# insight-platform/Similari

Hardware: NVIDIA H100
Metric: pair_associations_per_sec (higher is better)
Workload: dtype f32

## Files before the change

similari_b200/csrc/kernels_feat_tc.cu:

```cuda
#include <cuda.h>
#include <cuda_bf16.h>
#include <cuda_runtime.h>
#include <stdint.h>

#include <algorithm>
#include <cstdlib>
#include <cstring>

#include "sb_engine.cuh"
#include "sb_tc.cuh"

namespace sb {

constexpr int TC_STAGES = 4;
constexpr int TC_STAGE_BYTES = TC_A_BYTES + TC_B_BYTES;

struct TcHdr { int scene, m0, ncols_left, m, det_base, col0, epoch, vis_lbase, vis_lcap, pad; };
struct TcSmem {
  unsigned char stage[TC_STAGES][TC_STAGE_BYTES];
  VisColMeta meta[4][TC_BN];
  VisRowMeta rowm[4][TC_BM];
  float colb[4][TC_BN];
  unsigned int colvalid[4][TC_BN / 32];
  TcHdr hdr[4];
// ... 149 lines not shown
        const int total = __shfl_sync(0xffffffffu, incl, 31);
        int base = 0;
        if (lane == 31) base = atomicAdd(&f.vis_cnt[h.scene], total);
        base = __shfl_sync(0xffffffffu, base, 31);
        int pos = base + incl - cnt;
#pragma unroll
        for (int hr = 0; hr < 2; ++hr) {
#pragma unroll
          for (int w = 0; w < 4; ++w) {
            unsigned int kk = keep[w] & (hr ? 0xccccccccu : 0x33333333u);
            while (kk) {
              const int b = __ffs(kk) - 1;
              kk &= kk - 1;
              if (pos < h.vis_lcap) {
                const int i = w * 32 + b;
                const VisColMeta cm = gmeta[8 * (i >> 2) + q2 + (i & 1)];
                VisPair vp;
                vp.g = g[hr]; vp.row = cm.row; vp.scene = h.scene; vp.outcol = cm.outcol;
                f.vis_pairs[h.vis_lbase + pos] = vp;
              }
              ++pos;
            }
          }
        }
      }
      __syncwarp();
      if (lane == 0) mbar_arrive(&S.meta_empty[ms]);
    }
  }
  __syncthreads();
  cluster_sync_all();
}

constexpr int SA_BN = 128;
constexpr int SA_KMAX = 8;
constexpr int SA_A_BLOCK = TC_BM * TC_BK * 2;
constexpr int SA_B_STAGE = SA_BN * TC_BK * 2;
constexpr int SA_STAGES = 5;
constexpr int SA_SLABS = 4;
struct SaHdr { int scene, m0, ncols, m, det_base, col0, epoch, vis_lbase, vis_lcap, unit, last, pad; };
struct SaSmem {
  unsigned char a[SA_KMAX][SA_A_BLOCK];
  unsigned char b[SA_STAGES][SA_B_STAGE];
  VisColMeta meta[SA_SLABS][SA_BN];
  float colb[SA_SLABS][SA_BN];
  unsigned int colvalid[SA_SLABS][SA_BN / 32];
  SaHdr hdr[SA_SLABS];
  unsigned long long a_full[SA_KMAX];
  unsigned long long a_empty;
  unsigned long long full_bar[SA_STAGES];
  unsigned long long empty_bar[SA_STAGES];
  unsigned long long meta_full[SA_SLABS];
  unsigned long long meta_empty[SA_SLABS];
};
static_assert(sizeof(SaSmem) + 1024 <= 227 * 1024, "A-stationary screen kernel exceeds the shared memory of an SM");
constexpr int kScreenStationaryMaxD8 = SA_KMAX * TC_BK;

template <bool COSINE>
__global__ void __launch_bounds__(TC_THREADS, 1)
vis_screen_sa_kernel(const __grid_constant__ CUtensorMap mapA, const __grid_constant__ CUtensorMap mapB, Params p,
                     TrackStore ts, Frame f, const TcTile* units, int n_units_host, const int* n_units_dev, int ucols,
                     const VisColMeta* colmeta, const VisColGeo* colgeo, const VisRowMeta* rowmeta, const float* colb,
                     const unsigned int* colvalid) {
  const int n_units = n_units_dev ? *n_units_dev : n_units_host;
  extern __shared__ unsigned char smem_raw_[];
  SaSmem& S = *reinterpret_cast<SaSmem*>(smem_raw_ + ((1024u - (smem_u32(smem_raw_) & 1023u)) & 1023u));
  const int warp = threadIdx.x >> 5, lane = threadIdx.x & 31;
  const int K = p.max_obs;
  const int KB = (p.d8 + TC_BK - 1) / TC_BK;
  const uint32_t crank = cluster_rank();
  if (threadIdx.x == 0) {
    for (int kb = 0; kb < SA_KMAX; ++kb) mbar_init(&S.a_full[kb], 1);
    mbar_init(&S.a_empty, 2);
    for (int s = 0; s < SA_STAGES; ++s) { mbar_init(&S.full_bar[s], 1); mbar_init(&S.empty_bar[s], 2); }
    for (int b = 0; b < SA_SLABS; ++b) { mbar_init(&S.meta_full[b], 1); mbar_init(&S.meta_empty[b], 4); }
    asm volatile("fence.mbarrier_init.release.cluster;" ::: "memory");
  }
  __syncthreads();
  cluster_sync_all();

  if (warp < 4) {
    asm volatile("setmaxnreg.dec.sync.aligned.u32 40;");
    if (warp == 0 && lane == 0) {
      asm volatile("prefetch.tensormap [%0];" ::"l"((uint64_t)&mapA) : "memory");
      asm volatile("prefetch.tensormap [%0];" ::"l"((uint64_t)&mapB) : "memory");
      int seq = 0, gk = 0, unit = 0;
      for (int u = (int)(blockIdx.x >> 1); u < n_units; u += (int)(gridDim.x >> 1), ++unit) {
        const TcTile tl = units[u];
        const SceneDesc sc = f.scenes[tl.scene];
        const int m0 = tl.m0 + (int)crank * TC_BM;
        const int rowA = sc.det_base + m0;
        const int cols = min(ucols, sc.nb * K - tl.c0);
        const int nct = (cols + SA_BN - 1) / SA_BN;
        const int rowB = sc.slot * ts.track_cap * K + tl.c0;
        if (unit > 0) mbar_wait(&S.a_empty, (unit - 1) & 1);
        if (nct == 1) mbar_arrive(&S.a_empty);
        for (int ct = 0; ct < nct; ++ct, ++seq) {
          const int g = seq % SA_SLABS;
          mbar_wait(&S.meta_empty[g], ((seq / SA_SLABS) & 1) ^ 1);
          SaHdr h;
          h.scene = tl.scene; h.m0 = m0; h.ncols = min(SA_BN, cols - ct * SA_BN); h.m = sc.m; h.det_base = sc.det_base;
          h.col0 = sc.col_off + tl.c0 + ct * SA_BN; h.epoch = (int)sc.epoch; h.vis_lbase = sc.vis_lbase;
          h.vis_lcap = sc.vis_lcap; h.unit = unit; h.last = ct + 2 >= nct; h.pad = 0;
          S.hdr[g] = h;
          mbar_expect_tx(&S.meta_full[g], (uint32_t)(sizeof(VisColMeta) * SA_BN + 4 * SA_BN + SA_BN / 8));
          bulk_load(S.meta[g], colmeta + h.col0, (uint32_t)(sizeof(VisColMeta) * SA_BN), &S.meta_full[g]);
          bulk_load(S.colb[g], colb + h.col0, 4 * SA_BN, &S.meta_full[g]);
          bulk_load(S.colvalid[g], colvalid + (h.col0 >> 5), SA_BN / 8, &S.meta_full[g]);
          for (int kb = 0; kb < KB; ++kb, ++gk) {
            if (ct == 0) {
              mbar_expect_tx(&S.a_full[kb], SA_A_BLOCK);
              tma_load_2d(S.a[kb], &mapA, kb * TC_BK, rowA, &S.a_full[kb]);
            }
            const int s = gk % SA_STAGES;
            mbar_wait(&S.empty_bar[s], ((gk / SA_STAGES) & 1) ^ 1);
            mbar_expect_tx(&S.full_bar[s], SA_B_STAGE);
            tma_load_2d_mc(S.b[s] + crank * (SA_B_STAGE / 2), &mapB, kb * TC_BK, rowB + ct * SA_BN + (int)crank * (SA_BN / 2),
                           &S.full_bar[s], (uint16_t)0x3);
          }
        }
      }
      for (int e = 0; e < 2; ++e, ++seq) {
        const int g = seq % SA_SLABS;
        mbar_wait(&S.meta_empty[g], ((seq / SA_SLABS) & 1) ^ 1);
        S.hdr[g].scene = -1 - e;
        mbar_arrive(&S.meta_full[g]);
      }
    }
  } else {
    asm volatile("setmaxnreg.inc.sync.aligned.u32 232;");
    const int wg = (warp >> 2) - 1;
    const int rr[2] = {(warp & 3) * 16 + (lane >> 2), (warp & 3) * 16 + (lane >> 2) + 8};
    const int q2 = 2 * (lane & 3);
    const bool geo = p.n_constraints > 0;
    const bool elected = (threadIdx.x & 127) == 0;
    for (int pos = wg;; pos += 2) {
      const int ms = pos % SA_SLABS;
      mbar_wait(&S.meta_full[ms], (pos / SA_SLABS) & 1);
      const SaHdr h = S.hdr[ms];
      if (pos > 0) wg2_bar_sync(1 + (pos & 1));
      if (h.scene < 0) {
        if (h.scene == -1) wg2_bar_arrive(1 + ((pos + 1) & 1));
        break;
      }
      float rowk[2][2];
      bool row_ok[2][2];
#pragma unroll
      for (int hh = 0; hh < 2; ++hh)
#pragma unroll
        for (int hr = 0; hr < 2; ++hr) {
          const int m = h.m0 + 64 * hh + rr[hr];
          const VisRowMeta rm = rowmeta[h.det_base + m];
          rowk[hh][hr] = rm.rowk;
          row_ok[hh][hr] = m < h.m && rm.ok;
        }

      float acc[128];
      {
        const int g0 = pos * KB;
        int stage = g0 % SA_STAGES;
        uint32_t phase = (g0 / SA_STAGES) & 1;
        int prev = -1;
        auto release = [&](int s) {
          if (elected)
            for (uint32_t r = 0; r < 2; ++r) mbar_arrive_cluster(cluster_addr(&S.empty_bar[s], r));
        };
        for (int kb = 0; kb < KB; ++kb) {
          mbar_wait(&S.a_full[kb], (uint32_t)h.unit & 1u);
          mbar_wait(&S.full_bar[stage], phase);
          const uint32_t a0 = smem_u32(S.a[kb]);
          const uint32_t b0 = smem_u32(S.b[stage]);
          wgmma_fence();
#pragma unroll
          for (int k = 0; k < TC_BK / 16; ++k) {
            const uint32_t acc_on = (kb | k) != 0 ? 1u : 0u;
// ... 43 lines not shown
        keep[2 * hh + 1] &= colm[1] & rowm;
      }
      if (geo) {
        float cx[2][2], cy[2][2], cr[2][2];
#pragma unroll
        for (int hh = 0; hh < 2; ++hh)
#pragma unroll
          for (int hr = 0; hr < 2; ++hr) {
            cx[hh][hr] = 0.0f; cy[hh][hr] = 0.0f; cr[hh][hr] = 0.0f;
            if (row_ok[hh][hr]) {
              const size_t g = (size_t)h.det_base + h.m0 + 64 * hh + rr[hr];
              cx[hh][hr] = f.c_box[g * 6]; cy[hh][hr] = f.c_box[g * 6 + 1]; cr[hh][hr] = f.c_radius[g];
            }
          }
#pragma unroll
        for (int w = 0; w < 4; ++w) {
          unsigned int kk = keep[w];
          while (kk) {
            const int b = __ffs(kk) - 1;
            kk &= kk - 1;
            const int i = (w & 1) * 32 + b, hh = w >> 1;
            const bool r8 = (i >> 1) & 1;
            const int col = 8 * (i >> 2) + q2 + (i & 1);
            const VisColGeo cg = colgeo[h.col0 + col];
            if (!compat_ok(p, (unsigned int)h.epoch, cg.tep, r8 ? cx[hh][1] : cx[hh][0], r8 ? cy[hh][1] : cy[hh][0],
                           r8 ? cr[hh][1] : cr[hh][0], cg.tx, cg.ty, cg.tr))
              keep[w] &= ~(1u << b);
          }
        }
      }
      int cnt = 0;
#pragma unroll
      for (int w = 0; w < 4; ++w) cnt += __popc(keep[w]);
      if (__any_sync(0xffffffffu, cnt != 0)) {
        int incl = cnt;
#pragma unroll
        for (int o = 1; o < 32; o <<= 1) {
          int tt = __shfl_up_sync(0xffffffffu, incl, o);
          if (lane >= o) incl += tt;
        }
        const int total = __shfl_sync(0xffffffffu, incl, 31);
        int base = 0;
        if (lane == 31) base = atomicAdd(&f.vis_cnt[h.scene], total);
        base = __shfl_sync(0xffffffffu, base, 31);
        int at = base + incl - cnt;
#pragma unroll
        for (int hh = 0; hh < 2; ++hh) {
#pragma unroll
          for (int hr = 0; hr < 2; ++hr) {
            const int g = h.det_base + h.m0 + 64 * hh + rr[hr];
#pragma unroll
            for (int w = 0; w < 2; ++w) {
              unsigned int kk = keep[2 * hh + w] & (hr ? 0xccccccccu : 0x33333333u);
              while (kk) {
                const int b = __ffs(kk) - 1;
                kk &= kk - 1;
                if (at < h.vis_lcap) {
                  const int i = w * 32 + b;
                  const VisColMeta cm = gmeta[8 * (i >> 2) + q2 + (i & 1)];
                  VisPair vp;
                  vp.g = g; vp.row = cm.row; vp.scene = h.scene; vp.outcol = cm.outcol;
                  f.vis_pairs[h.vis_lbase + at] = vp;
                }
                ++at;
              }
            }
          }
        }
      }
      __syncwarp();
      if (lane == 0) mbar_arrive(&S.meta_empty[ms]);
    }
  }
  __syncthreads();
  cluster_sync_all();
}

__device__ __forceinline__ float reduce_add8_tc(const float* t) {
  float q0 = t[0] + t[4], q1 = t[1] + t[5], q2 = t[2] + t[6], q3 = t[3] + t[7];
  float d0 = q0 + q2, d1 = q1 + q3;
  return d0 + d1;
}

constexpr int RF_WARPS = 4;
constexpr int RF_SEG = 64;
constexpr int RF_PITCH = RF_SEG + 1;

template <bool TAIL>
__device__ __forceinline__ void refine_load_a(const float* __restrict__ a, int blk, int D, float* av) {
  if (!TAIL) {
    const float4 a0 = *reinterpret_cast<const float4*>(a + blk * 8);
    const float4 a1 = *reinterpret_cast<const float4*>(a + blk * 8 + 4);
    av[0] = a0.x; av[1] = a0.y; av[2] = a0.z; av[3] = a0.w; av[4] = a1.x; av[5] = a1.y; av[6] = a1.z; av[7] = a1.w;
  } else {
#pragma unroll
    for (int l = 0; l < 8; ++l) av[l] = blk * 8 + l < D ? a[blk * 8 + l] : 0.0f;
  }
}
template <bool COSINE>
__device__ __forceinline__ float refine_block_sum(const float* av, const float* __restrict__ b, int blk) {
  const float4 b0 = *reinterpret_cast<const float4*>(b + blk * 8);
  const float4 b1 = *reinterpret_cast<const float4*>(b + blk * 8 + 4);
  const float bb[8] = {b0.x, b0.y, b0.z, b0.w, b1.x, b1.y, b1.z, b1.w};
  float t[8];
#pragma unroll
  for (int l = 0; l < 8; ++l) {
    if (COSINE) t[l] = av[l] * bb[l];
    else { const float df = av[l] - bb[l]; t[l] = df * df; }
  }
  return reduce_add8_tc(t);
}

template <bool COSINE, bool TAIL, int RP>
__global__ void __launch_bounds__(RF_WARPS * 32, RP == 32 ? 6 : 8) vis_refine_kernel(Params p, TrackStore ts, Frame f, int* nan_flag) {
  __shared__ float s_bs[RF_WARPS][RP][RF_PITCH];
  const int scene = blockIdx.y;
  if (f.vis_mode[scene] != 0) return;
  const SceneDesc sc = f.scenes[scene];
  const int lane = threadIdx.x & 31, w = threadIdx.x >> 5;
  const int n_pairs = min(f.vis_cnt[scene], sc.vis_lcap);
  const int nblk = p.d8 / 8;
  const int D = p.feature_dim;
  float (*bs)[RF_PITCH] = s_bs[w];
  float vmax = nanf("");
  for (;;) {
    int i0 = 0;
    if (lane == 0) i0 = atomicAdd(f.refine_next + scene, RP);
    i0 = __shfl_sync(0xffffffffu, i0, 0);
    if (i0 >= n_pairs) break;
    const int npair = min(RP, n_pairs - i0);
    VisPair mine;
    mine.g = 0; mine.row = 0; mine.scene = 0; mine.outcol = 0;
    if (lane < npair) mine = f.vis_pairs[sc.vis_lbase + i0 + lane];
    float acc = 0.0f;
    for (int seg0 = 0; seg0 < nblk; seg0 += RF_SEG) {
      const int segn = min(RF_SEG, nblk - seg0);
      int g_prev = -1;
      float av[RF_SEG / 32][8];
#pragma unroll 4
      for (int pp = 0; pp < npair; ++pp) {
        const int g = __shfl_sync(0xffffffffu, mine.g, pp);
        const int row = __shfl_sync(0xffffffffu, mine.row, pp);
        const float* b = ts.feat + (size_t)row * p.d8;
        if (g != g_prev) {
          const float* a = f.in_feat + (size_t)g * D;
#pragma unroll
          for (int h = 0; h < RF_SEG / 32; ++h)
            if (h * 32 + lane < segn) refine_load_a<TAIL>(a, seg0 + h * 32 + lane, D, av[h]);
          g_prev = g;
        }
#pragma unroll
        for (int h = 0; h < RF_SEG / 32; ++h) {
          const int j = h * 32 + lane;
          if (j < segn) bs[pp][j] = refine_block_sum<COSINE>(av[h], b, seg0 + j);
        }
      }
      __syncwarp();
      if (lane < npair)
        for (int j = 0; j < segn; ++j) acc = acc + bs[lane][j];
      __syncwarp();
    }
    if (lane < npair) {
      float v = nanf("");
      if (COSINE) {
        const float d = acc / sqrtf(f.c_norm2[mine.g] * ts.fnorm2[mine.row]);
        if (d >= p.visual_threshold) v = 1.0f - d;
      } else {
        const float d = sqrtf(acc);
        if (d <= p.visual_threshold) v = d;
      }
      f.vis_val[sc.vis_lbase + i0 + lane] = v;
      if (!is_nan(v) && !(v <= vmax)) vmax = v;
      if (nan_flag && is_nan(v)) nan_flag[scene] = 1;
    }
  }
  unsigned int u = 0u;
  if (!is_nan(vmax)) {
    u = __float_as_uint(vmax);
    u = (u & 0x80000000u) ? ~u : (u | 0x80000000u);
  }
#pragma unroll
  for (int o = 16; o > 0; o >>= 1) u = max(u, __shfl_xor_sync(0xffffffffu, u, o));
  if (lane == 0 && u != 0u) atomicMax(f.scene_max + scene, u);
}

constexpr int RA_WARPS = 6;
constexpr int RA_STAGES = 3;
constexpr int RA_PAIRS = 2;
constexpr int RA_SEGF = RF_SEG * 8;
constexpr int RA_STAGE_FLOATS = RA_PAIRS * 2 * RA_SEGF;

__device__ __forceinline__ void cp_async16(void* smem_dst, const void* gsrc) {
  asm volatile("cp.async.cg.shared.global [%0], [%1], 16;" ::"r"(smem_u32(smem_dst)), "l"(gsrc) : "memory");
}
__device__ __forceinline__ void cp_async_commit() { asm volatile("cp.async.commit_group;" ::: "memory"); }
template <int N>
__device__ __forceinline__ void cp_async_wait() { asm volatile("cp.async.wait_group %0;" ::"n"(N) : "memory"); }

template <bool COSINE>
__global__ void __launch_bounds__(RA_WARPS * 32) vis_refine_async_kernel(Params p, TrackStore ts, Frame f, int* nan_flag) {
  extern __shared__ __align__(16) unsigned char ra_smem[];
  const int scene = blockIdx.y;
  if (f.vis_mode[scene] != 0) return;
  const SceneDesc sc = f.scenes[scene];
  const int lane = threadIdx.x & 31, w = threadIdx.x >> 5;
  float* stage0 = reinterpret_cast<float*>(ra_smem) + (size_t)w * (RA_STAGES * RA_STAGE_FLOATS + 32 * RF_PITCH);
  float (*bs)[RF_PITCH] = reinterpret_cast<float (*)[RF_PITCH]>(stage0 + RA_STAGES * RA_STAGE_FLOATS);
  const int n_pairs = min(f.vis_cnt[scene], sc.vis_lcap);
  const int nblk = p.d8 / 8;
  const int D = p.feature_dim;
  float vmax = nanf("");
  for (;;) {
    int i0 = 0;
    if (lane == 0) i0 = atomicAdd(f.refine_next + scene, 32);
    i0 = __shfl_sync(0xffffffffu, i0, 0);
    if (i0 >= n_pairs) break;
// ... 45 lines not shown
          const int pp = st * RA_PAIRS + pi;
          if (pp < npair) {
            const float* sa = src + (pi * 2) * RA_SEGF;
            const float* sb2 = sa + RA_SEGF;
#pragma unroll
            for (int h = 0; h < RF_SEG / 32; ++h) {
              const int j = h * 32 + lane;
              if (j < segn) {
                const float4 a0 = *reinterpret_cast<const float4*>(sa + j * 4);
                const float4 a1 = *reinterpret_cast<const float4*>(sa + (RF_SEG + j) * 4);
                const float4 b0 = *reinterpret_cast<const float4*>(sb2 + j * 4);
                const float4 b1 = *reinterpret_cast<const float4*>(sb2 + (RF_SEG + j) * 4);
                const float av[8] = {a0.x, a0.y, a0.z, a0.w, a1.x, a1.y, a1.z, a1.w};
                const float bv[8] = {b0.x, b0.y, b0.z, b0.w, b1.x, b1.y, b1.z, b1.w};
                float t[8];
#pragma unroll
                for (int l = 0; l < 8; ++l) {
                  if (COSINE) t[l] = av[l] * bv[l];
                  else { const float df = av[l] - bv[l]; t[l] = df * df; }
                }
                bs[pp][j] = reduce_add8_tc(t);
              }
            }
          }
        }
        __syncwarp();
      }
      cp_async_wait<0>();
      if (lane < npair)
        for (int j = 0; j < segn; ++j) acc = acc + bs[lane][j];
      __syncwarp();
    }
    if (lane < npair) {
      float v = nanf("");
      if (COSINE) {
        const float d = acc / sqrtf(f.c_norm2[mine.g] * ts.fnorm2[mine.row]);
        if (d >= p.visual_threshold) v = 1.0f - d;
      } else {
        const float d = sqrtf(acc);
        if (d <= p.visual_threshold) v = d;
      }
      f.vis_val[sc.vis_lbase + i0 + lane] = v;
      if (!is_nan(v) && !(v <= vmax)) vmax = v;
      if (nan_flag && is_nan(v)) nan_flag[scene] = 1;
    }
  }
  unsigned int u = 0u;
  if (!is_nan(vmax)) {
    u = __float_as_uint(vmax);
    u = (u & 0x80000000u) ? ~u : (u | 0x80000000u);
  }
#pragma unroll
  for (int o = 16; o > 0; o >>= 1) u = max(u, __shfl_xor_sync(0xffffffffu, u, o));
  if (lane == 0 && u != 0u) atomicMax(f.scene_max + scene, u);
}

__global__ void vis_fill_none_kernel(Params p, Frame f) {
  const int scene = blockIdx.y;
  if (f.scene_mode[scene] != 0) return;
  const SceneDesc sc = f.scenes[scene];
  const long long cnt = (long long)sc.m * sc.n * p.max_obs;
  float* out = f.vis + sc.vis_off;
  const float qnan = nanf("");
  for (long long i = (long long)blockIdx.x * blockDim.x + threadIdx.x; i < cnt; i += (long long)gridDim.x * blockDim.x) out[i] = qnan;
}
__global__ void vis_scatter_kernel(Params p, Frame f) {
  const int scene = blockIdx.y;
  if (f.scene_mode[scene] != 0) return;
  const SceneDesc sc = f.scenes[scene];
  const int n_pairs = min(f.vis_cnt[scene], sc.vis_lcap);
  float* out = f.vis + sc.vis_off;
  for (int i = blockIdx.x * blockDim.x + threadIdx.x; i < n_pairs; i += gridDim.x * blockDim.x) {
    const VisPair vp = f.vis_pairs[sc.vis_lbase + i];
    out[(size_t)(vp.g - sc.det_base) * (sc.n * p.max_obs) + vp.outcol] = f.vis_val[sc.vis_lbase + i];
  }
}
void launch_vis_densify(const Params& p, const Frame& f, int n_scenes, cudaStream_t st) {
  if (n_scenes == 0) return;
  dim3 grid(64, n_scenes);
  vis_fill_none_kernel<<<grid, 256, 0, st>>>(p, f);
  vis_scatter_kernel<<<grid, 256, 0, st>>>(p, f);
  note_launch(2);
}

__global__ void to_bf16_kernel(const float* src, int src_pitch, int d, int d8, long long rows, __nv_bfloat16* dst) {
  long long i = (long long)blockIdx.x * blockDim.x + threadIdx.x;
  if (i >= rows * d8) return;
// ... 77 lines not shown
        for (int k = 0; k < K; ++k) {
          bool lv = k < on && ts.obs_hasf[ti * K + k];
          if (!lv) { if (seen == dead_rank) { cm.outcol = n * K + k; break; } ++seen; }
        }
      }
    }
    colmeta[sc.col_off + prow] = cm;
    colb[sc.col_off + prow] = cm.colb;
    if (p.n_constraints > 0) {
      VisColGeo cg;
      cg.tx = 0.0f; cg.ty = 0.0f; cg.tr = 0.0f; cg.tep = tep;
      if (n >= 0) { const float* tb = ts.pred + ti * 6; cg.tx = tb[0]; cg.ty = tb[1]; cg.tr = ts.radius[ti]; }
      colgeo[sc.col_off + prow] = cg;
    }
  }
  const unsigned int vb = __ballot_sync(0xffffffffu, cm.row >= 0);
  if ((threadIdx.x & 31) == 0 && vb != 0) colvalid[(sc.col_off + prow) >> 5] = vb;
  else if ((threadIdx.x & 31) == 0 && in) colvalid[(sc.col_off + prow) >> 5] = 0u;
}

__global__ void vis_rowmeta_kernel(Params p, Frame f, VisRowMeta* rowmeta) {
  int g = blockIdx.x * blockDim.x + threadIdx.x;
  if (g >= f.total) return;
  g += f.det0;
  const float na = f.c_norm2[g];
  VisRowMeta rm;
  rm.ok = (f.c_flags[g] & 2) ? 1 : 0;
  const float thr = p.visual_threshold;
  if (p.visual_kind == 1) rm.rowk = (thr - 1e-5f - kScreenRelErr) * sqrtf(na);
  else rm.rowk = 0.5f * (na * (1.0f - 1e-5f - kScreenRelErr) - thr * thr * (1.0f + 1e-5f));
  rowmeta[g] = rm;
}

int launch_vis_refine(const Params& p, const TrackStore& ts, const Frame& f, int n_scenes, int* nan_flag, cudaStream_t st) {
  if (n_scenes == 0) return 0;
  dim3 grid(16, n_scenes);
  const bool tail = p.feature_dim != p.d8 || (reinterpret_cast<uintptr_t>(f.in_feat) & 15) != 0;
  static const bool async_copy = getenv("SB200_REFINE") != nullptr && !strcmp(getenv("SB200_REFINE"), "async");
  if (!tail && async_copy) {
    const size_t smem = (size_t)RA_WARPS * (RA_STAGES * RA_STAGE_FLOATS + 32 * RF_PITCH) * sizeof(float);
    const void* fn = p.visual_kind == 1 ? (const void*)vis_refine_async_kernel<true> : (const void*)vis_refine_async_kernel<false>;
    cudaError_t e = cudaFuncSetAttribute(fn, cudaFuncAttributeMaxDynamicSharedMemorySize, (int)smem);
    if (e != cudaSuccess) return (int)e;
    dim3 grid2(8, n_scenes);
    if (p.visual_kind == 1) vis_refine_async_kernel<true><<<grid2, RA_WARPS * 32, smem, st>>>(p, ts, f, nan_flag);
    else vis_refine_async_kernel<false><<<grid2, RA_WARPS * 32, smem, st>>>(p, ts, f, nan_flag);
    note_launch();
    return 0;
  }
  static const bool rp16 = !(getenv("SB200_REFINE_PAIRS") != nullptr && atoi(getenv("SB200_REFINE_PAIRS")) == 32);
#define SB_RF(C, T)                                                                        \
  do {                                                                                     \
    if (rp16) vis_refine_kernel<C, T, 16><<<grid, RF_WARPS * 32, 0, st>>>(p, ts, f, nan_flag); \
    else vis_refine_kernel<C, T, 32><<<grid, RF_WARPS * 32, 0, st>>>(p, ts, f, nan_flag);      \
  } while (0)
  if (p.visual_kind == 1) {
    if (tail) SB_RF(true, true); else SB_RF(true, false);
  } else {
    if (tail) SB_RF(false, true); else SB_RF(false, false);
  }
#undef SB_RF
  note_launch();
  return 0;
}

void launch_vis_colmeta(const Params& p, const TrackStore& ts, const Frame& f, int n_scenes, int max_n, const TcArgs& tc,
                        cudaStream_t st) {
  const int max_rows = tc.max_rows > 0 ? tc.max_rows : max_n * p.max_obs;
  if (tc.n_tiles == 0 || max_rows <= 0) return;
  dim3 grid((max_rows + 255) / 256, n_scenes);
  vis_meta_kernel<<<grid, 256, 0, st>>>(p, ts, f, n_scenes, max_rows, tc.colmeta, tc.colgeo, tc.colb, tc.colvalid);
  note_launch();
}

int vis_screen_ucols(int d8, int num_sms, int n_scenes, const int* m, const int* nb, int K) {
  if (d8 > kScreenStationaryMaxD8) return TC_BN;
  long long pairs = 0, pair_tiles = 0;
  int max_ct = 1;
  for (int s = 0; s < n_scenes; ++s) {
    const int ct = (nb[s] * K + SA_BN - 1) / SA_BN, rp = (m[s] + 2 * TC_BM - 1) / (2 * TC_BM);
    pairs += rp;
    pair_tiles += (long long)rp * ct;
    max_ct = std::max(max_ct, ct);
  }
  const long long units = 2ll * std::max(1, num_sms / 2);
  if (pairs >= units) return max_ct * SA_BN;
  const long long per = (pair_tiles + units - 1) / units;
  return (int)std::max<long long>(2, std::min<long long>(per, max_ct)) * SA_BN;
}

int launch_vis_cost_tc(const Params& p, const TrackStore& ts, const Frame& f, int n_scenes, int max_n, const TcArgs& tc,
                       int phase, cudaStream_t st) {
  if (tc.n_tiles == 0) return 0;
  if (phase == 1) {
    int rc = launch_vis_refine(p, ts, f, n_scenes, nullptr, st);
    if (tc.ev_refine1) cudaEventRecord(tc.ev_refine1, st);
    return rc;
  }
  const bool stationary = p.d8 <= kScreenStationaryMaxD8;
  CUtensorMap mA, mB;
  if (make_map(&mA, f.c_bf16, tc.a_rows, p.d8, TC_BM) ||
      make_map(&mB, ts.feat_bf16, tc.b_rows, p.d8, stationary ? SA_BN / 2 : TC_BN / 2))
    return -1;
  const size_t smem = (stationary ? sizeof(SaSmem) : sizeof(TcSmem)) + 1024;
  const bool cosine = p.visual_kind == 1;
  cudaError_t e = cudaSuccess;
  const void* fn = stationary ? (cosine ? (const void*)vis_screen_sa_kernel<true> : (const void*)vis_screen_sa_kernel<false>)
                              : (cosine ? (const void*)vis_screen_kernel<true> : (const void*)vis_screen_kernel<false>);
  e = cudaFuncSetAttribute(fn, cudaFuncAttributeMaxDynamicSharedMemorySize, (int)smem);
  if (e != cudaSuccess) return (int)e;
  if (!tc.colmeta_done) launch_vis_colmeta(p, ts, f, n_scenes, max_n, tc, st);
  vis_rowmeta_kernel<<<(f.total + 255) / 256, 256, 0, st>>>(p, f, tc.rowmeta);
  note_launch();
  if (tc.ev_screen0) cudaEventRecord(tc.ev_screen0, st);
  {
    const int ncta = 2 * std::min(tc.n_tiles, tc.num_sms / 2);
    cudaLaunchConfig_t cfg;
    memset(&cfg, 0, sizeof(cfg));
    cfg.gridDim = dim3(ncta);
    cfg.blockDim = dim3(TC_THREADS);
    cfg.dynamicSmemBytes = smem;
    cfg.stream = st;
    cudaLaunchAttribute attr[1];
    attr[0].id = cudaLaunchAttributeClusterDimension;
    attr[0].val.clusterDim.x = 2; attr[0].val.clusterDim.y = 1; attr[0].val.clusterDim.z = 1;
    cfg.attrs = attr;
    cfg.numAttrs = 1;
    const TcTile* d_tiles = tc.d_tiles;
    int n_tiles = tc.n_tiles;
    const int* d_n_tiles = tc.d_n_tiles;
    const VisColMeta* cmeta = tc.colmeta;
    const VisColGeo* cgeo = tc.colgeo;
    const VisRowMeta* rmeta = tc.rowmeta;
    const float* cb = tc.colb;
    const unsigned int* cv = tc.colvalid;
    int ucols = tc.cstep;
    void* args[] = {(void*)&mA, (void*)&mB, (void*)&p, (void*)&ts, (void*)&f, (void*)&d_tiles, (void*)&n_tiles,
                    (void*)&d_n_tiles, (void*)&cmeta, (void*)&cgeo, (void*)&rmeta, (void*)&cb, (void*)&cv};
    void* args_sa[] = {(void*)&mA, (void*)&mB, (void*)&p, (void*)&ts, (void*)&f, (void*)&d_tiles, (void*)&n_tiles,
                       (void*)&d_n_tiles, (void*)&ucols, (void*)&cmeta, (void*)&cgeo, (void*)&rmeta, (void*)&cb, (void*)&cv};
    e = cudaLaunchKernelExC(&cfg, fn, stationary ? args_sa : args);
    if (e != cudaSuccess) return (int)e;
    note_launch();
  }
  if (tc.ev_screen1) cudaEventRecord(tc.ev_screen1, st);
  return 0;
}

}
```

similari_b200/csrc/sb_tc.cuh:

```cuda
#pragma once
#include <cuda.h>
#include <cuda_runtime.h>
#include <stdint.h>

namespace sb {

constexpr int TC_BM = 128, TC_BN = 256, TC_BK = 64;
constexpr int TC_A_BYTES = TC_BM * TC_BK * 2;
constexpr int TC_B_BYTES = TC_BN * TC_BK * 2;
constexpr int TC_WG_ROWS = 64;
constexpr int TC_THREADS = 384;

__device__ __forceinline__ uint32_t smem_u32(const void* p) { return (uint32_t)__cvta_generic_to_shared(p); }
__device__ __forceinline__ void mbar_init(void* bar, uint32_t count) {
  asm volatile("mbarrier.init.shared::cta.b64 [%0], %1;" ::"r"(smem_u32(bar)), "r"(count));
}
__device__ __forceinline__ void mbar_expect_tx(void* bar, uint32_t bytes) {
  asm volatile("mbarrier.arrive.expect_tx.shared::cta.b64 _, [%0], %1;" ::"r"(smem_u32(bar)), "r"(bytes) : "memory");
}
__device__ __forceinline__ void mbar_arrive(void* bar) {
  asm volatile("mbarrier.arrive.shared::cta.b64 _, [%0];" ::"r"(smem_u32(bar)) : "memory");
}
__device__ __forceinline__ void mbar_wait(void* bar, uint32_t parity) {
  uint32_t done;
// ... 5 lines not shown
        "selp.u32 %0, 1, 0, P1;\n\t"
        "}" : "=r"(done) : "r"(smem_u32(bar)), "r"(parity) : "memory");
  } while (!done);
}
__device__ __forceinline__ void tma_load_2d(void* dst, const CUtensorMap* map, int c0, int c1, void* bar) {
  asm volatile(
      "cp.async.bulk.tensor.2d.shared::cluster.global.mbarrier::complete_tx::bytes [%0], [%1, {%3, %4}], [%2];"
      ::"r"(smem_u32(dst)), "l"((uint64_t)map), "r"(smem_u32(bar)), "r"(c0), "r"(c1) : "memory");
}
__device__ __forceinline__ void tma_load_2d_mc(void* dst, const CUtensorMap* map, int c0, int c1, void* bar, uint16_t mask) {
  asm volatile(
      "cp.async.bulk.tensor.2d.shared::cluster.global.mbarrier::complete_tx::bytes.multicast::cluster [%0], [%1, {%4, %5}], [%2], %3;"
      ::"r"(smem_u32(dst)), "l"((uint64_t)map), "r"(smem_u32(bar)), "h"(mask), "r"(c0), "r"(c1) : "memory");
}
__device__ __forceinline__ uint32_t cluster_addr(const void* p, uint32_t rank) {
  uint32_t r;
  asm volatile("mapa.shared::cluster.u32 %0, %1, %2;" : "=r"(r) : "r"(smem_u32(p)), "r"(rank));
  return r;
}
__device__ __forceinline__ void mbar_arrive_cluster(uint32_t cluster_bar) {
  asm volatile("mbarrier.arrive.shared::cluster.b64 _, [%0];" ::"r"(cluster_bar) : "memory");
}
__device__ __forceinline__ uint32_t cluster_rank() {
  uint32_t r;
  asm volatile("mov.u32 %0, %%cluster_ctarank;" : "=r"(r));
  return r;
}
__device__ __forceinline__ void cluster_sync_all() {
  asm volatile("barrier.cluster.arrive.release.aligned;\n\tbarrier.cluster.wait.acquire.aligned;" ::: "memory");
}
__device__ __forceinline__ void bulk_load(void* dst, const void* src, uint32_t bytes, void* bar) {
  asm volatile("cp.async.bulk.shared::cluster.global.mbarrier::complete_tx::bytes [%0], [%1], %2, [%3];"
               ::"r"(smem_u32(dst)), "l"((uint64_t)src), "r"(bytes), "r"(smem_u32(bar)) : "memory");
}
__device__ __forceinline__ void wg_bar(int id) { asm volatile("bar.sync %0, 128;" ::"r"(id) : "memory"); }
__device__ __forceinline__ void wg2_bar_sync(int id) { asm volatile("bar.sync %0, 256;" ::"r"(id) : "memory"); }
__device__ __forceinline__ void wg2_bar_arrive(int id) { asm volatile("bar.arrive %0, 256;" ::"r"(id) : "memory"); }

__device__ __forceinline__ void wgmma_fence() { asm volatile("wgmma.fence.sync.aligned;" ::: "memory"); }
__device__ __forceinline__ void wgmma_commit() { asm volatile("wgmma.commit_group.sync.aligned;" ::: "memory"); }
template <int N>
__device__ __forceinline__ void wgmma_wait() { asm volatile("wgmma.wait_group.sync.aligned %0;" ::"n"(N) : "memory"); }
__device__ __forceinline__ void wgmma_bf16_m64n256(float* d, uint64_t adesc, uint64_t bdesc, uint32_t accum) {
  asm volatile(
      "{\n\t"
      ".reg .pred p;\n\t"
      "setp.ne.b32 p, %130, 0;\n\t"
      "wgmma.mma_async.sync.aligned.m64n256k16.f32.bf16.bf16 {"
      "%0, %1, %2, %3, %4, %5, %6, %7, %8, %9, %10, %11, %12, %13, %14, %15, %16, %17, %18, %19, %20, %21, %22, %23, %24, %25, %26, %27, %28, %29, %30, %31, "
      "%32, %33, %34, %35, %36, %37, %38, %39, %40, %41, %42, %43, %44, %45, %46, %47, %48, %49, %50, %51, %52, %53, %54, %55, %56, %57, %58, %59, %60, %61, %62, %63, "
      "%64, %65, %66, %67, %68, %69, %70, %71, %72, %73, %74, %75, %76, %77, %78, %79, %80, %81, %82, %83, %84, %85, %86, %87, %88, %89, %90, %91, %92, %93, %94, %95, "
      "%96, %97, %98, %99, %100, %101, %102, %103, %104, %105, %106, %107, %108, %109, %110, %111, %112, %113, %114, %115, %116, %117, %118, %119, %120, %121, %122, %123, %124, %125, %126, %127 "
      "}, %128, %129, p, 1, 1, 0, 0;\n\t"
      "}"
      : "+f"(d[0]), "+f"(d[1]), "+f"(d[2]), "+f"(d[3]), "+f"(d[4]), "+f"(d[5]), "+f"(d[6]), "+f"(d[7]), "+f"(d[8]), "+f"(d[9]), "+f"(d[10]), "+f"(d[11]), "+f"(d[12]), "+f"(d[13]), "+f"(d[14]), "+f"(d[15]),
        "+f"(d[16]), "+f"(d[17]), "+f"(d[18]), "+f"(d[19]), "+f"(d[20]), "+f"(d[21]), "+f"(d[22]), "+f"(d[23]), "+f"(d[24]), "+f"(d[25]), "+f"(d[26]), "+f"(d[27]), "+f"(d[28]), "+f"(d[29]), "+f"(d[30]), "+f"(d[31]),
        "+f"(d[32]), "+f"(d[33]), "+f"(d[34]), "+f"(d[35]), "+f"(d[36]), "+f"(d[37]), "+f"(d[38]), "+f"(d[39]), "+f"(d[40]), "+f"(d[41]), "+f"(d[42]), "+f"(d[43]), "+f"(d[44]), "+f"(d[45]), "+f"(d[46]), "+f"(d[47]),
        "+f"(d[48]), "+f"(d[49]), "+f"(d[50]), "+f"(d[51]), "+f"(d[52]), "+f"(d[53]), "+f"(d[54]), "+f"(d[55]), "+f"(d[56]), "+f"(d[57]), "+f"(d[58]), "+f"(d[59]), "+f"(d[60]), "+f"(d[61]), "+f"(d[62]), "+f"(d[63]),
        "+f"(d[64]), "+f"(d[65]), "+f"(d[66]), "+f"(d[67]), "+f"(d[68]), "+f"(d[69]), "+f"(d[70]), "+f"(d[71]), "+f"(d[72]), "+f"(d[73]), "+f"(d[74]), "+f"(d[75]), "+f"(d[76]), "+f"(d[77]), "+f"(d[78]), "+f"(d[79]),
        "+f"(d[80]), "+f"(d[81]), "+f"(d[82]), "+f"(d[83]), "+f"(d[84]), "+f"(d[85]), "+f"(d[86]), "+f"(d[87]), "+f"(d[88]), "+f"(d[89]), "+f"(d[90]), "+f"(d[91]), "+f"(d[92]), "+f"(d[93]), "+f"(d[94]), "+f"(d[95]),
        "+f"(d[96]), "+f"(d[97]), "+f"(d[98]), "+f"(d[99]), "+f"(d[100]), "+f"(d[101]), "+f"(d[102]), "+f"(d[103]), "+f"(d[104]), "+f"(d[105]), "+f"(d[106]), "+f"(d[107]), "+f"(d[108]), "+f"(d[109]), "+f"(d[110]), "+f"(d[111]),
        "+f"(d[112]), "+f"(d[113]), "+f"(d[114]), "+f"(d[115]), "+f"(d[116]), "+f"(d[117]), "+f"(d[118]), "+f"(d[119]), "+f"(d[120]), "+f"(d[121]), "+f"(d[122]), "+f"(d[123]), "+f"(d[124]), "+f"(d[125]), "+f"(d[126]), "+f"(d[127])
      : "l"(adesc), "l"(bdesc), "r"(accum));
}
__device__ __forceinline__ void wgmma_bf16_m64n128(float* d, uint64_t adesc, uint64_t bdesc, uint32_t accum) {
  asm volatile(
// ... 64 lines not shown
```

Baseline: 53.26 billion.

## Fuse exact refine pass into A-stationary screen kernel using idle producer warps

Warps 1-3 of the producer warpgroup, previously idle, now act as refine workers. Consumer warpgroups push each slab's surviving candidate ranges into an mbarrier-guarded shared-memory queue, and the refine warps compute exact fp32 distances, write vis_val and update the scene max. L2 bulk prefetch of the feature rows is added. The separate refine kernel launch is skipped when the screen kernel handles refinement. Register budgets are rebalanced (producer raised to 96, consumers lowered to 200), which could cause consumer spills, and queue back-pressure could stall the MMA warps.

```diff
diff --git a/similari_b200/csrc/kernels_feat_tc.cu b/similari_b200/csrc/kernels_feat_tc.cu
--- a/similari_b200/csrc/kernels_feat_tc.cu
+++ b/similari_b200/csrc/kernels_feat_tc.cu
@@ -205,13 +205,76 @@
   cluster_sync_all();
 }
 
+constexpr int RF_SEG = 64;
+constexpr int RF_PITCH = RF_SEG + 1;
+
+__device__ __forceinline__ float reduce_add8_tc(const float* t) {
+  float q0 = t[0] + t[4], q1 = t[1] + t[5], q2 = t[2] + t[6], q3 = t[3] + t[7];
+  float d0 = q0 + q2, d1 = q1 + q3;
+  return d0 + d1;
+}
+template <bool TAIL>
+__device__ __forceinline__ void refine_load_a(const float* __restrict__ a, int blk, int D, float* av) {
+  if (!TAIL) {
+    const float4 a0 = *reinterpret_cast<const float4*>(a + blk * 8);
+    const float4 a1 = *reinterpret_cast<const float4*>(a + blk * 8 + 4);
+    av[0] = a0.x; av[1] = a0.y; av[2] = a0.z; av[3] = a0.w; av[4] = a1.x; av[5] = a1.y; av[6] = a1.z; av[7] = a1.w;
+  } else {
+#pragma unroll
+    for (int l = 0; l < 8; ++l) av[l] = blk * 8 + l < D ? a[blk * 8 + l] : 0.0f;
+  }
+}
+template <bool COSINE>
+__device__ __forceinline__ float refine_block_sum(const float* av, const float* bb) {
+  float t[8];
+#pragma unroll
+  for (int l = 0; l < 8; ++l) {
+    if (COSINE) t[l] = av[l] * bb[l];
+    else { const float df = av[l] - bb[l]; t[l] = df * df; }
+  }
+  return reduce_add8_tc(t);
+}
+template <bool COSINE>
+__device__ __forceinline__ float refine_block_sum(const float* av, const float* __restrict__ b, int blk) {
+  const float4 b0 = *reinterpret_cast<const float4*>(b + blk * 8);
+  const float4 b1 = *reinterpret_cast<const float4*>(b + blk * 8 + 4);
+  const float bb[8] = {b0.x, b0.y, b0.z, b0.w, b1.x, b1.y, b1.z, b1.w};
+  return refine_block_sum<COSINE>(av, bb);
+}
+template <bool COSINE>
+__device__ __forceinline__ float refine_value(const Params& p, const TrackStore& ts, const Frame& f, float acc, int g, int row) {
+  float v = nanf("");
+  if (COSINE) {
+    const float d = acc / sqrtf(f.c_norm2[g] * ts.fnorm2[row]);
+    if (d >= p.visual_threshold) v = 1.0f - d;
+  } else {
+    const float d = sqrtf(acc);
+    if (d <= p.visual_threshold) v = d;
+  }
+  return v;
+}
+__device__ __forceinline__ void refine_max_flush(const Frame& f, int scene, float vmax) {
+  unsigned int u = 0u;
+  if (!is_nan(vmax)) {
+    u = __float_as_uint(vmax);
+    u = (u & 0x80000000u) ? ~u : (u | 0x80000000u);
+  }
+#pragma unroll
+  for (int o = 16; o > 0; o >>= 1) u = max(u, __shfl_xor_sync(0xffffffffu, u, o));
+  if ((threadIdx.x & 31) == 0 && u != 0u) atomicMax(f.scene_max + scene, u);
+}
+
 constexpr int SA_BN = 128;
 constexpr int SA_KMAX = 8;
 constexpr int SA_A_BLOCK = TC_BM * TC_BK * 2;
 constexpr int SA_B_STAGE = SA_BN * TC_BK * 2;
 constexpr int SA_STAGES = 5;
 constexpr int SA_SLABS = 4;
+constexpr int SA_RWARPS = 3;
+constexpr int SA_RQ = 8;
+constexpr int SA_RP = 8;
 struct SaHdr { int scene, m0, ncols, m, det_base, col0, epoch, vis_lbase, vis_lcap, unit, last, pad; };
+struct SaRefineEntry { int scene, lbase, base[4], cnt[4]; };
 struct SaSmem {
   unsigned char a[SA_KMAX][SA_A_BLOCK];
   unsigned char b[SA_STAGES][SA_B_STAGE];
@@ -219,13 +282,31 @@
   float colb[SA_SLABS][SA_BN];
   unsigned int colvalid[SA_SLABS][SA_BN / 32];
   SaHdr hdr[SA_SLABS];
+  SaRefineEntry rq[SA_RQ];
+  float rbs[SA_RWARPS][SA_RP][RF_PITCH];
   unsigned long long a_full[SA_KMAX];
   unsigned long long a_empty;
   unsigned long long full_bar[SA_STAGES];
   unsigned long long empty_bar[SA_STAGES];
   unsigned long long meta_full[SA_SLABS];
   unsigned long long meta_empty[SA_SLABS];
+  unsigned long long rq_full[SA_RQ];
+  unsigned long long rq_empty[SA_RQ];
 };
+
+__device__ __forceinline__ void refine_push(SaSmem& S, int pos, int scene, int lbase, int base, int cnt) {
+  const int qs = pos % SA_RQ, w = (threadIdx.x >> 5) & 3;
+  if ((threadIdx.x & 31) == 0) {
+    mbar_wait(&S.rq_empty[qs], ((pos / SA_RQ) & 1) ^ 1);
+    SaRefineEntry& e = S.rq[qs];
+    e.scene = scene;
+    e.lbase = lbase;
+    e.base[w] = base;
+    e.cnt[w] = cnt;
+    mbar_arrive(&S.rq_full[qs]);
+  }
+  __syncwarp();
+}
 static_assert(sizeof(SaSmem) + 1024 <= 227 * 1024, "A-stationary screen kernel exceeds the shared memory of an SM");
 constexpr int kScreenStationaryMaxD8 = SA_KMAX * TC_BK;
 
@@ -234,7 +315,7 @@
 vis_screen_sa_kernel(const __grid_constant__ CUtensorMap mapA, const __grid_constant__ CUtensorMap mapB, Params p,
                      TrackStore ts, Frame f, const TcTile* units, int n_units_host, const int* n_units_dev, int ucols,
                      const VisColMeta* colmeta, const VisColGeo* colgeo, const VisRowMeta* rowmeta, const float* colb,
-                     const unsigned int* colvalid) {
+                     const unsigned int* colvalid, int refine) {
   const int n_units = n_units_dev ? *n_units_dev : n_units_host;
   extern __shared__ unsigned char smem_raw_[];
   SaSmem& S = *reinterpret_cast<SaSmem*>(smem_raw_ + ((1024u - (smem_u32(smem_raw_) & 1023u)) & 1023u));
@@ -247,14 +328,94 @@
     mbar_init(&S.a_empty, 2);
     for (int s = 0; s < SA_STAGES; ++s) { mbar_init(&S.full_bar[s], 1); mbar_init(&S.empty_bar[s], 2); }
     for (int b = 0; b < SA_SLABS; ++b) { mbar_init(&S.meta_full[b], 1); mbar_init(&S.meta_empty[b], 4); }
+    for (int q = 0; q < SA_RQ; ++q) { mbar_init(&S.rq_full[q], 4); mbar_init(&S.rq_empty[q], 1); }
     asm volatile("fence.mbarrier_init.release.cluster;" ::: "memory");
   }
   __syncthreads();
   cluster_sync_all();
 
   if (warp < 4) {
-    asm volatile("setmaxnreg.dec.sync.aligned.u32 40;");
-    if (warp == 0 && lane == 0) {
+    asm volatile("setmaxnreg.dec.sync.aligned.u32 96;");
+    if (warp >= 1 && refine) {
+      const int r = warp - 1;
+      float (*bs)[RF_PITCH] = S.rbs[r];
+      const int nblk = p.d8 / 8;
+      const int D = p.feature_dim;
+      for (int pos = r;; pos += SA_RWARPS) {
+        const int qs = pos % SA_RQ;
+        mbar_wait(&S.rq_full[qs], (pos / SA_RQ) & 1);
+        const SaRefineEntry& e = S.rq[qs];
+        const int scene = e.scene, lbase = e.lbase;
+        if (scene < 0) break;
+        const int n = e.cnt[0] + e.cnt[1] + e.cnt[2] + e.cnt[3];
+        float vmax = nanf("");
+        for (int k0 = 0; k0 < n; k0 += 32) {
+          const int npair = min(32, n - k0);
+          int at = -1;
+          VisPair mine;
+          mine.g = 0; mine.row = 0; mine.scene = 0; mine.outcol = 0;
+          if (lane < npair) {
+            int kk = k0 + lane;
+#pragma unroll
+            for (int w = 0; w < 4; ++w) {
+              const int c = e.cnt[w];
+              if (at < 0 && kk < c) at = e.base[w] + kk;
+              kk -= c;
+            }
+            mine = f.vis_pairs[lbase + at];
+            bulk_prefetch_l2(ts.feat + (size_t)mine.row * p.d8, (uint32_t)p.d8 * 4u);
+          }
+          const int g_up = __shfl_up_sync(0xffffffffu, mine.g, 1);
+          if (lane < npair && (lane == 0 || g_up != mine.g)) bulk_prefetch_l2(f.in_feat + (size_t)mine.g * D, (uint32_t)D * 4u);
+          for (int p0 = 0; p0 < npair; p0 += SA_RP) {
+            const int gn = min(SA_RP, npair - p0);
+            for (int pp = 0; pp < gn; pp += 2) {
+              const int q1 = min(pp + 1, gn - 1);
+              const float* a[2];
+              const float* b[2];
+#pragma unroll
+              for (int u = 0; u < 2; ++u) {
+                const int src = p0 + (u ? q1 : pp);
+                a[u] = f.in_feat + (size_t)__shfl_sync(0xffffffffu, mine.g, src) * D;
+                b[u] = ts.feat + (size_t)__shfl_sync(0xffffffffu, mine.row, src) * p.d8;
+              }
+              float av[2][RF_SEG / 32][8], bv[2][RF_SEG / 32][8];
+#pragma unroll
+              for (int u = 0; u < 2; ++u)
+#pragma unroll
+                for (int h = 0; h < RF_SEG / 32; ++h) {
+                  const int j = min(h * 32 + lane, nblk - 1);
+                  refine_load_a<false>(a[u], j, D, av[u][h]);
+                  refine_load_a<false>(b[u], j, D, bv[u][h]);
+                }
+#pragma unroll
+              for (int u = 0; u < 2; ++u)
+#pragma unroll
+                for (int h = 0; h < RF_SEG / 32; ++h) {
+                  const int j = h * 32 + lane;
+                  if (j < nblk && (u == 0 || q1 != pp)) bs[u ? q1 : pp][j] = refine_block_sum<COSINE>(av[u][h], bv[u][h]);
+                }
+            }
+            __syncwarp();
+            const int src = (p0 + lane) & 31;
+            const int g = __shfl_sync(0xffffffffu, mine.g, src);
+            const int row = __shfl_sync(0xffffffffu, mine.row, src);
+            const int ati = __shfl_sync(0xffffffffu, at, src);
+            if (lane < gn) {
+              float acc = 0.0f;
+              for (int j = 0; j < nblk; ++j) acc = acc + bs[lane][j];
+              const float v = refine_value<COSINE>(p, ts, f, acc, g, row);
+              f.vis_val[lbase + ati] = v;
+              if (!is_nan(v) && !(v <= vmax)) vmax = v;
+            }
+            __syncwarp();
+          }
+        }
+        __syncwarp();
+        if (lane == 0) mbar_arrive(&S.rq_empty[qs]);
+        refine_max_flush(f, scene, vmax);
+      }
+    } else if (warp == 0 && lane == 0) {
       asm volatile("prefetch.tensormap [%0];" ::"l"((uint64_t)&mapA) : "memory");
       asm volatile("prefetch.tensormap [%0];" ::"l"((uint64_t)&mapB) : "memory");
       int seq = 0, gk = 0, unit = 0;
@@ -301,7 +462,7 @@
       }
     }
   } else {
-    asm volatile("setmaxnreg.inc.sync.aligned.u32 232;");
+    asm volatile("setmaxnreg.inc.sync.aligned.u32 200;");
     const int wg = (warp >> 2) - 1;
     const int rr[2] = {(warp & 3) * 16 + (lane >> 2), (warp & 3) * 16 + (lane >> 2) + 8};
     const int q2 = 2 * (lane & 3);
@@ -314,6 +475,10 @@
       if (pos > 0) wg2_bar_sync(1 + (pos & 1));
       if (h.scene < 0) {
         if (h.scene == -1) wg2_bar_arrive(1 + ((pos + 1) & 1));
+        if (refine) {
+          refine_push(S, pos, -1, 0, 0, 0);
+          if (h.scene == -1) refine_push(S, pos + 2, -1, 0, 0, 0);
+        }
         break;
       }
       float rowk[2][2];
@@ -423,6 +588,7 @@
       int cnt = 0;
 #pragma unroll
       for (int w = 0; w < 4; ++w) cnt += __popc(keep[w]);
+      int base = 0, total = 0;
       if (__any_sync(0xffffffffu, cnt != 0)) {
         int incl = cnt;
 #pragma unroll
@@ -430,8 +596,7 @@
           int tt = __shfl_up_sync(0xffffffffu, incl, o);
           if (lane >= o) incl += tt;
         }
-        const int total = __shfl_sync(0xffffffffu, incl, 31);
-        int base = 0;
+        total = __shfl_sync(0xffffffffu, incl, 31);
         if (lane == 31) base = atomicAdd(&f.vis_cnt[h.scene], total);
         base = __shfl_sync(0xffffffffu, base, 31);
         int at = base + incl - cnt;
@@ -461,46 +626,14 @@
       }
       __syncwarp();
       if (lane == 0) mbar_arrive(&S.meta_empty[ms]);
+      if (refine) refine_push(S, pos, h.scene, h.vis_lbase, base, max(0, min(total, h.vis_lcap - base)));
     }
   }
   __syncthreads();
   cluster_sync_all();
 }
 
-__device__ __forceinline__ float reduce_add8_tc(const float* t) {
-  float q0 = t[0] + t[4], q1 = t[1] + t[5], q2 = t[2] + t[6], q3 = t[3] + t[7];
-  float d0 = q0 + q2, d1 = q1 + q3;
-  return d0 + d1;
-}
-
 constexpr int RF_WARPS = 4;
-constexpr int RF_SEG = 64;
-constexpr int RF_PITCH = RF_SEG + 1;
-
-template <bool TAIL>
-__device__ __forceinline__ void refine_load_a(const float* __restrict__ a, int blk, int D, float* av) {
-  if (!TAIL) {
-    const float4 a0 = *reinterpret_cast<const float4*>(a + blk * 8);
-    const float4 a1 = *reinterpret_cast<const float4*>(a + blk * 8 + 4);
-    av[0] = a0.x; av[1] = a0.y; av[2] = a0.z; av[3] = a0.w; av[4] = a1.x; av[5] = a1.y; av[6] = a1.z; av[7] = a1.w;
-  } else {
-#pragma unroll
-    for (int l = 0; l < 8; ++l) av[l] = blk * 8 + l < D ? a[blk * 8 + l] : 0.0f;
-  }
-}
-template <bool COSINE>
-__device__ __forceinline__ float refine_block_sum(const float* av, const float* __restrict__ b, int blk) {
-  const float4 b0 = *reinterpret_cast<const float4*>(b + blk * 8);
-  const float4 b1 = *reinterpret_cast<const float4*>(b + blk * 8 + 4);
-  const float bb[8] = {b0.x, b0.y, b0.z, b0.w, b1.x, b1.y, b1.z, b1.w};
-  float t[8];
-#pragma unroll
-  for (int l = 0; l < 8; ++l) {
-    if (COSINE) t[l] = av[l] * bb[l];
-    else { const float df = av[l] - bb[l]; t[l] = df * df; }
-  }
-  return reduce_add8_tc(t);
-}
 
 template <bool COSINE, bool TAIL, int RP>
 __global__ void __launch_bounds__(RF_WARPS * 32, RP == 32 ? 6 : 8) vis_refine_kernel(Params p, TrackStore ts, Frame f, int* nan_flag) {
@@ -552,27 +685,13 @@
       __syncwarp();
     }
     if (lane < npair) {
-      float v = nanf("");
-      if (COSINE) {
-        const float d = acc / sqrtf(f.c_norm2[mine.g] * ts.fnorm2[mine.row]);
-        if (d >= p.visual_threshold) v = 1.0f - d;
-      } else {
-        const float d = sqrtf(acc);
-        if (d <= p.visual_threshold) v = d;
-      }
+      const float v = refine_value<COSINE>(p, ts, f, acc, mine.g, mine.row);
       f.vis_val[sc.vis_lbase + i0 + lane] = v;
       if (!is_nan(v) && !(v <= vmax)) vmax = v;
       if (nan_flag && is_nan(v)) nan_flag[scene] = 1;
     }
   }
-  unsigned int u = 0u;
-  if (!is_nan(vmax)) {
-    u = __float_as_uint(vmax);
-    u = (u & 0x80000000u) ? ~u : (u | 0x80000000u);
-  }
-#pragma unroll
-  for (int o = 16; o > 0; o >>= 1) u = max(u, __shfl_xor_sync(0xffffffffu, u, o));
-  if (lane == 0 && u != 0u) atomicMax(f.scene_max + scene, u);
+  refine_max_flush(f, scene, vmax);
 }
 
 constexpr int RA_WARPS = 6;
@@ -684,27 +803,13 @@
       __syncwarp();
     }
     if (lane < npair) {
-      float v = nanf("");
-      if (COSINE) {
-        const float d = acc / sqrtf(f.c_norm2[mine.g] * ts.fnorm2[mine.row]);
-        if (d >= p.visual_threshold) v = 1.0f - d;
-      } else {
-        const float d = sqrtf(acc);
-        if (d <= p.visual_threshold) v = d;
-      }
+      const float v = refine_value<COSINE>(p, ts, f, acc, mine.g, mine.row);
       f.vis_val[sc.vis_lbase + i0 + lane] = v;
       if (!is_nan(v) && !(v <= vmax)) vmax = v;
       if (nan_flag && is_nan(v)) nan_flag[scene] = 1;
     }
   }
-  unsigned int u = 0u;
-  if (!is_nan(vmax)) {
-    u = __float_as_uint(vmax);
-    u = (u & 0x80000000u) ? ~u : (u | 0x80000000u);
-  }
-#pragma unroll
-  for (int o = 16; o > 0; o >>= 1) u = max(u, __shfl_xor_sync(0xffffffffu, u, o));
-  if (lane == 0 && u != 0u) atomicMax(f.scene_max + scene, u);
+  refine_max_flush(f, scene, vmax);
 }
 
 __global__ void vis_fill_none_kernel(Params p, Frame f) {
@@ -848,10 +953,17 @@
   rowmeta[g] = rm;
 }
 
+static bool refine_tail(const Params& p, const Frame& f) {
+  return p.feature_dim != p.d8 || (reinterpret_cast<uintptr_t>(f.in_feat) & 15) != 0;
+}
+static bool screen_refines(const Params& p, const Frame& f) {
+  return p.d8 <= kScreenStationaryMaxD8 && !refine_tail(p, f);
+}
+
 int launch_vis_refine(const Params& p, const TrackStore& ts, const Frame& f, int n_scenes, int* nan_flag, cudaStream_t st) {
   if (n_scenes == 0) return 0;
   dim3 grid(16, n_scenes);
-  const bool tail = p.feature_dim != p.d8 || (reinterpret_cast<uintptr_t>(f.in_feat) & 15) != 0;
+  const bool tail = refine_tail(p, f);
   static const bool async_copy = getenv("SB200_REFINE") != nullptr && !strcmp(getenv("SB200_REFINE"), "async");
   if (!tail && async_copy) {
     const size_t smem = (size_t)RA_WARPS * (RA_STAGES * RA_STAGE_FLOATS + 32 * RF_PITCH) * sizeof(float);
@@ -909,7 +1021,8 @@
                        int phase, cudaStream_t st) {
   if (tc.n_tiles == 0) return 0;
   if (phase == 1) {
-    int rc = launch_vis_refine(p, ts, f, n_scenes, nullptr, st);
+    int rc = 0;
+    if (tc.dense || !screen_refines(p, f)) rc = launch_vis_refine(p, ts, f, n_scenes, nullptr, st);
     if (tc.ev_refine1) cudaEventRecord(tc.ev_refine1, st);
     return rc;
   }
@@ -951,10 +1064,12 @@
     const float* cb = tc.colb;
     const unsigned int* cv = tc.colvalid;
     int ucols = tc.cstep;
+    int refine = screen_refines(p, f) ? 1 : 0;
     void* args[] = {(void*)&mA, (void*)&mB, (void*)&p, (void*)&ts, (void*)&f, (void*)&d_tiles, (void*)&n_tiles,
                     (void*)&d_n_tiles, (void*)&cmeta, (void*)&cgeo, (void*)&rmeta, (void*)&cb, (void*)&cv};
     void* args_sa[] = {(void*)&mA, (void*)&mB, (void*)&p, (void*)&ts, (void*)&f, (void*)&d_tiles, (void*)&n_tiles,
-                       (void*)&d_n_tiles, (void*)&ucols, (void*)&cmeta, (void*)&cgeo, (void*)&rmeta, (void*)&cb, (void*)&cv};
+                       (void*)&d_n_tiles, (void*)&ucols, (void*)&cmeta, (void*)&cgeo, (void*)&rmeta, (void*)&cb, (void*)&cv,
+                       (void*)&refine};
     e = cudaLaunchKernelExC(&cfg, fn, stationary ? args_sa : args);
     if (e != cudaSuccess) return (int)e;
     note_launch();
diff --git a/similari_b200/csrc/sb_tc.cuh b/similari_b200/csrc/sb_tc.cuh
--- a/similari_b200/csrc/sb_tc.cuh
+++ b/similari_b200/csrc/sb_tc.cuh
@@ -61,6 +61,9 @@
 __device__ __forceinline__ void bulk_load(void* dst, const void* src, uint32_t bytes, void* bar) {
   asm volatile("cp.async.bulk.shared::cluster.global.mbarrier::complete_tx::bytes [%0], [%1], %2, [%3];"
                ::"r"(smem_u32(dst)), "l"((uint64_t)src), "r"(bytes), "r"(smem_u32(bar)) : "memory");
+}
+__device__ __forceinline__ void bulk_prefetch_l2(const void* src, uint32_t bytes) {
+  asm volatile("cp.async.bulk.prefetch.L2.global [%0], %1;" ::"l"((uint64_t)src), "r"(bytes) : "memory");
 }
 __device__ __forceinline__ void wg_bar(int id) { asm volatile("bar.sync %0, 128;" ::"r"(id) : "memory"); }
 __device__ __forceinline__ void wg2_bar_sync(int id) { asm volatile("bar.sync %0, 256;" ::"r"(id) : "memory"); }
```

After: 53.63 billion (median of 6 runs). Within noise of the previous version (+0.7%).
